# NazirNayal8/RbA

Hardware: AMD Instinct MI355X
Metric: images/sec @1024x2048 Swin-B-1dl (RbA inference hot path) (higher is better)
Workload: dtype f32 (f16x3 split-MFMA GEMMs, fp32 accumulate)

## Files before the change

include/rba_hip.h:

```cpp
#ifndef RBA_HIP_H
#define RBA_HIP_H

#include <stdint.h>

#ifdef __cplusplus
extern "C" {
#endif

int rba_hip_version(void);

int rba_set_concurrent_streams(int n);

int rba_reduce_f32(const float* mask, const float* cls_prob, float* rba, float* sem_seg, int32_t* argmax,
                   int Q, int K, int64_t HW, int score_mode, void* stream);

int rba_reduce_ws_f32(const float* mask, const float* cls_prob, float* rba, float* sem_seg, int32_t* argmax, int Q, int K,
                      int64_t HW, int score_mode, void* workspace, void* stream);

int rba_reduce_up4_f32(const float* mask_lowres, const float* cls_prob, float* rba, float* sem_seg,
                       int32_t* argmax, int Q, int K, int h, int w, int crop_h, int crop_w, int score_mode, void* stream);

int rba_reduce_bwd_workspace_f32(int Q, int K, int64_t HW, int64_t* bytes);
int rba_reduce_bwd_f32(const float* mask, const float* cls_prob, const float* grad_score,
                       float* grad_mask , float* grad_prob ,
// ... 127 lines not shown
                                        int rows_per_image, void* stream);

int rba_split_linear_nchw_out_gn_f16x3_f32(const float* x, const float* mr, const float* gamma, const float* beta, int G, int relu,
                                           const void* weight_packed, const float* bias, float* out, int64_t M, int N, int K,
                                           int rows_per_image, void* stream);

int rba_split_linear_nchw_out_gn_rows_f16x3_f32(const float* x, const float* mr, const float* gamma, const float* beta, int G, int relu,
                                                const void* weight_packed, int64_t weight_image_stride, const float* bias,
                                                int bias_image_stride, const int32_t* row_index, float* out, int B, int P, int R, int N,
                                                int K, void* stream);
int rba_compose_query_operand_f16x2(const float* embed, const float* weight, const float* bias, void* packed, float* bias_q, int B, int Q,
                                    int C, int K, void* stream);

int rba_conv3x3_nhwc_f32(const float* x, const void* weight_packed, const float* bias, float* out, int B, int H, int W, int C,
                         int N, void* stream);

int rba_conv3x3_nhwc_f16x3_f32(const float* x, const void* weight_packed, const float* bias, float* out, int B, int H, int W, int C,
                               int N, void* stream);

int rba_split_linear_f16x3_gn_moments_f32(const float* x, const void* weight_packed, const float* bias, float* out, int64_t M, int N, int K,
                                          int rows_per_image, int G, float* moments, void* stream);
int rba_conv3x3_nhwc_f16x3_split_in_gn_moments_f32(const void* x_frag, const void* weight_packed, const float* bias, float* out, int B, int H,
                                                   int W, int C, int N, int G, float* moments, void* stream);
int rba_group_norm_nhwc_merge_f32(const float* moments, float* mr, int B, int G, int splits, float eps, void* stream);

int rba_patch_im2col_u8(const uint8_t* image, float* out, int h, int w, int Hp, int Wp, const float* mean, const float* std, void* stream);
int rba_patch_im2col_f32(const float* image, float* out, int h, int w, int Hp, int Wp, const float* mean, const float* std, void* stream);

int rba_gaussian_blur_f32(const float* in, float* out, int H, int W, int kernel_size, float sigma, void* stream);

int rba_quad_mean_f32(const float* v, float* out, int64_t rows, int S, void* stream);
int rba_softmax_drop_last_f32(const float* logits, float* prob, int64_t rows, int K1, void* stream);

int rba_threshold_u8(const float* score, uint8_t* out, int64_t n, float threshold, void* stream);
int rba_morph3x3_u8(const uint8_t* in, uint8_t* out, int H, int W, int dilate, void* stream);
int rba_ccl4_roots_i32(const uint8_t* mask, int32_t* roots, int H, int W, void* stream);

int rba_bn_relu_conv1x1_f32(const float* x, const float* scale, const float* shift, const float* weight, const float* bias, float* out,
                            int B, int C, int O, int64_t P, void* stream);
int rba_resample_bilinear_ac_f32(const float* x, float* out, int C, int h, int w, int H, int W, void* stream);

typedef struct {
  const float* x_add;
  const void* packed;
  const float* bias;
  float* out;
// ... 15 lines not shown
```

rba_amd/_lib.py:

```python
import ctypes
import os

_HERE = os.path.dirname(os.path.abspath(__file__))
LIB_PATH = os.environ.get("RBA_HIP_LIB") or os.path.join(_HERE, "csrc", "librba_hip.so")
KNOBS_LIB_PATH = os.path.join(_HERE, "csrc", "librba_hip_knobs.so")

_i = ctypes.c_int
_i64 = ctypes.c_int64
_vp = ctypes.c_void_p

SIGNATURES = {
    "rba_hip_version": [],
    "rba_set_concurrent_streams": [_i],
    "rba_reduce_f32": [_vp, _vp, _vp, _vp, _vp, _i, _i, _i64, _i, _vp],
    "rba_reduce_ws_f32": [_vp, _vp, _vp, _vp, _vp, _i, _i, _i64, _i, _vp, _vp],
    "rba_reduce_up4_f32": [_vp, _vp, _vp, _vp, _vp, _i, _i, _i, _i, _i, _i, _i, _vp],
    "rba_reduce_bwd_workspace_f32": [_i, _i, _i64, _vp],
    "rba_reduce_bwd_f32": [_vp, _vp, _vp, _vp, _vp, _i, _i, _i64, _i, _vp, _i64, _vp],
    "rba_resample_bilinear_f32": [_vp, _vp, _vp, _i, _i, _i, _i, _i, _vp],
    "rba_ms_deform_attn_fwd_f32": [_vp, _vp, _vp, _vp, _vp, _vp, _i, _i, _i, _i, _i, _i, _i, _vp],
    "rba_ms_deform_attn_fwd_f64": [_vp, _vp, _vp, _vp, _vp, _vp, _i, _i, _i, _i, _i, _i, _i, _vp],
    "rba_ms_deform_attn_bwd_f32": [_vp, _vp, _vp, _vp, _vp, _vp, _vp, _vp, _vp, _i, _i, _i, _i, _i, _i, _i, _vp],
    "rba_ms_deform_attn_bwd_f64": [_vp, _vp, _vp, _vp, _vp, _vp, _vp, _vp, _vp, _i, _i, _i, _i, _i, _i, _i, _vp],
    "rba_msda_prepare_f32": [_vp, _vp, _vp, _vp, _vp, _i64, _i, _i, _i, _vp],
# ... 16 lines not shown
    "rba_swin_bias_fragments_elems": [_i, _i],
    "rba_swin_attn_block_supported": [_i, _i],
    "rba_swin_attn_block_weight_bytes": [_i],
    "rba_swin_attn_qkv_supported": [_i, _i],
    "rba_swin_attn_qkv_split_out_f32": [_vp, _vp, _vp, _vp, ctypes.c_float, _vp, _vp, _vp, _i, _i, _i, _i, _i, _i, _vp],
    "rba_swin_attn_block_pack_f32": [_vp, _vp, _vp, _i, _vp],
    "rba_swin_attn_block_f32": [_vp, _vp, _vp, _vp, ctypes.c_float, _vp, _vp, _vp, _vp, _vp, _vp, ctypes.c_float, _i, _i, _i, _i, _i, _i, _vp],
    "rba_swin_bias_fragments_f32": [_vp, _vp, _i, _i, _vp],
    "rba_skinny_linear_f32": [_vp, _vp, _vp, _vp, _i, _i, _i, _i, _vp],
    "rba_skinny_linear_add_f32": [_vp, _vp, _i, _vp, _vp, _vp, _i, _i, _i, _i, _i, _vp],
    "rba_split_weight_bf16x3": [_vp, _vp, _i, _i, _vp],
    "rba_split_linear_f32": [_vp, _vp, _vp, _vp, _i64, _i, _i, _i, _vp],
    "rba_split_weight_f16x2": [_vp, _vp, _i, _i, _vp],
    "rba_split_linear_f16x3_f32": [_vp, _vp, _vp, _vp, _i64, _i, _i, _i, _vp],
    "rba_split_linear_f16x3_res_f32": [_vp, _vp, _vp, _vp, _vp, _i64, _i, _i, _vp],
    "rba_split_linear_f16x3_frag_f32": [_vp, _vp, _vp, _vp, _vp, _i64, _i, _i, _i, _vp],
    "rba_swin_mlp_fused_f16x3_f32": [_vp, _vp, _vp, _vp, _vp, _vp, _vp, _i64, _i, _i, _vp],
    "rba_swin_mlp_fused_ln_f16x3_f32": [_vp, _vp, _vp, ctypes.c_float, _vp, _vp, _vp, _vp, _i64, _i, _i, _vp],
    "rba_split_linear_f16x3_gelu_split_out": [_vp, _i, _vp, _vp, _vp, _i64, _i, _i, _vp],
    "rba_split_linear_nchw_out_f32": [_vp, _vp, _vp, _vp, _i64, _i, _i, _i, _vp],
    "rba_split_linear_nchw_out_f16x3_f32": [_vp, _vp, _vp, _vp, _i64, _i, _i, _i, _vp],
    "rba_split_linear_f16x3_gn_moments_f32": [_vp, _vp, _vp, _vp, _i64, _i, _i, _i, _i, _vp, _vp],
    "rba_conv3x3_nhwc_f16x3_split_in_gn_moments_f32": [_vp, _vp, _vp, _vp, _i, _i, _i, _i, _i, _i, _vp, _vp],
    "rba_group_norm_nhwc_merge_f32": [_vp, _vp, _i, _i, _i, ctypes.c_float, _vp],
    "rba_split_linear_nchw_out_gn_f16x3_f32": [_vp, _vp, _vp, _vp, _i, _i, _vp, _vp, _vp, _i64, _i, _i, _i, _vp],
    "rba_split_linear_nchw_out_gn_rows_f16x3_f32": [_vp, _vp, _vp, _vp, _i, _i, _vp, _i64, _vp, _i, _vp, _vp, _i, _i, _i, _i, _i, _vp],
    "rba_compose_query_operand_f16x2": [_vp, _vp, _vp, _vp, _vp, _i, _i, _i, _i, _vp],
    "rba_conv3x3_nhwc_f32": [_vp, _vp, _vp, _vp, _i, _i, _i, _i, _i, _vp],
    "rba_conv3x3_nhwc_f16x3_f32": [_vp, _vp, _vp, _vp, _i, _i, _i, _i, _i, _vp],
    "rba_conv3x3_nhwc_f16x3_split_in_f32": [_vp, _vp, _vp, _vp, _i, _i, _i, _i, _i, _vp],
    "rba_resample_bilinear_nhwc_split_out_f32": [_vp, _vp, _vp, _i, _i, _i, _i, _i, _i64, _vp],
    "rba_patch_im2col_u8": [_vp, _vp, _i, _i, _i, _i, _vp, _vp, _vp],
    "rba_patch_im2col_f32": [_vp, _vp, _i, _i, _i, _i, _vp, _vp, _vp],
    "rba_group_norm_nhwc_workspace_bytes": [_i, _i, _i, _i],
    "rba_group_norm_nhwc_f32": [_vp, _vp, _vp, _vp, _vp, _i, _i, _i, _i, ctypes.c_float, _i, _vp],
    "rba_resample_bilinear_nhwc_f32": [_vp, _vp, _vp, _i, _i, _i, _i, _i, _vp],
    "rba_bn_relu_conv1x1_f32": [_vp, _vp, _vp, _vp, _vp, _vp, _i, _i, _i, _i64, _vp],
    "rba_resample_bilinear_ac_f32": [_vp, _vp, _i, _i, _i, _i, _i, _vp],
    "rba_gaussian_blur_f32": [_vp, _vp, _i, _i, _i, ctypes.c_float, _vp],
    "rba_quad_mean_f32": [_vp, _vp, _i64, _i, _vp],
    "rba_softmax_drop_last_f32": [_vp, _vp, _i64, _i, _vp],
    "rba_threshold_u8": [_vp, _vp, _i64, ctypes.c_float, _vp],
    "rba_morph3x3_u8": [_vp, _vp, _i, _i, _i, _vp],
    "rba_ccl4_roots_i32": [_vp, _vp, _i, _i, _vp],
    "rba_add_layer_norm_f32": [_vp, _vp, _vp, _vp, _vp, _vp, _vp, _i64, _i, ctypes.c_float, _vp],
    "rba_add_layer_norm_frag_f32": [_vp, _vp, _vp, _vp, _vp, _vp, _vp, _i64, _i, ctypes.c_float, _vp],
# ... 96 lines not shown
```

rba_amd/csrc/group_norm.hip:

```cpp
#include "common.h"
#include "../../include/rba_hip.h"

namespace {

constexpr int CHUNK = 16384;

__device__ __forceinline__ double wave_sum_d(double v) {
#pragma unroll
  for (int o = 32; o > 0; o >>= 1) v += __shfl_xor(v, o, RBA_WAVE);
  return v;
}

__global__ __launch_bounds__(256) void gn_stats_kernel(const float* __restrict__ x, float* __restrict__ ws, int64_t gsize,
                                                       int splits) {
  const int s = blockIdx.x, g = blockIdx.y;
  const int64_t lo = (int64_t)s * CHUNK, hi = lo + CHUNK < gsize ? lo + CHUNK : gsize;
  const float* p = x + (int64_t)g * gsize;
  float sum = 0.f, sq = 0.f;
  if ((gsize & 3) == 0 && (((uintptr_t)p) & 15) == 0) {
    for (int64_t i = lo + threadIdx.x * 4; i < hi; i += 1024) {
      const float4 v = *reinterpret_cast<const float4*>(p + i);
      sum += (v.x + v.y) + (v.z + v.w);
      sq = fmaf(v.x, v.x, sq); sq = fmaf(v.y, v.y, sq); sq = fmaf(v.z, v.z, sq); sq = fmaf(v.w, v.w, sq);
    }
// ... 77 lines not shown
    for (int p = lo + pl; p < hi; p += lanes) {
      const float4 v = xp[(int64_t)p * C4];
      sum += (v.x + v.y) + (v.z + v.w);
      sq = fmaf(v.x, v.x, sq); sq = fmaf(v.y, v.y, sq); sq = fmaf(v.z, v.z, sq); sq = fmaf(v.w, v.w, sq);
    }
  __shared__ float sh_s[256], sh_q[256];
  sh_s[threadIdx.x] = sum;
  sh_q[threadIdx.x] = sq;
  __syncthreads();
  const int G = C / cpg, q4 = cpg >> 2;
  if (threadIdx.x < G) {
    const int g = threadIdx.x;
    double ds = 0, dq = 0;
    for (int l = 0; l < lanes; ++l)
      for (int k = 0; k < q4; ++k) { ds += sh_s[l * C4 + g * q4 + k]; dq += sh_q[l * C4 + g * q4 + k]; }
    const double n = (double)(hi - lo) * cpg;
    const double mean = ds / n;
    const double m2 = dq - ds * mean;
    float* o = ws + (((int64_t)b * G + g) * splits + s) * 3;
    o[0] = (float)n; o[1] = (float)mean; o[2] = (float)(m2 > 0 ? m2 : 0);
  }
}

__global__ __launch_bounds__(64) void gn_merge_kernel(const float* __restrict__ ws, float* __restrict__ mr, int splits, float eps) {
  const float* w = ws + (int64_t)blockIdx.x * splits * 3;
  double n = 0, nm = 0;
  for (int i = threadIdx.x; i < splits; i += 64) { n += w[3 * i]; nm += (double)w[3 * i] * w[3 * i + 1]; }
  n = wave_sum_d(n); nm = wave_sum_d(nm);
  const double mean = nm / n;
  double m2 = 0;
  for (int i = threadIdx.x; i < splits; i += 64) {
    const double d = (double)w[3 * i + 1] - mean;
    m2 += (double)w[3 * i + 2] + (double)w[3 * i] * d * d;
  }
  m2 = wave_sum_d(m2);
  if (threadIdx.x == 0) { mr[2 * blockIdx.x] = (float)mean; mr[2 * blockIdx.x + 1] = (float)(1.0 / sqrt(m2 / n + (double)eps)); }
}

template <bool RELU>
__global__ __launch_bounds__(256) void gn_apply_nhwc_kernel(const float* __restrict__ x, const float* __restrict__ mr,
                                                            const float* __restrict__ gamma, const float* __restrict__ beta,
                                                            float* __restrict__ y, int P, int C, int cpg) {
  const int s = blockIdx.x, b = blockIdx.y;
  const int C4 = C >> 2, lanes = 256 / C4;
  const int j = threadIdx.x % C4, pl = threadIdx.x / C4;
  if (pl >= lanes) return;
  const int G = C / cpg, g = (j << 2) / cpg;
  const float mean = mr[2 * (b * G + g)], rstd = mr[2 * (b * G + g) + 1];
  const float4 ga = reinterpret_cast<const float4*>(gamma)[j], be = reinterpret_cast<const float4*>(beta)[j];
  const float a0 = ga.x * rstd, a1 = ga.y * rstd, a2 = ga.z * rstd, a3 = ga.w * rstd;
  const float b0 = fmaf(-mean, a0, be.x), b1 = fmaf(-mean, a1, be.y), b2 = fmaf(-mean, a2, be.z), b3 = fmaf(-mean, a3, be.w);
  const int lo = s * PIX_CHUNK, hi = lo + PIX_CHUNK < P ? lo + PIX_CHUNK : P;
  const float4* xp = reinterpret_cast<const float4*>(x + (int64_t)b * P * C) + j;
  float4* yp = reinterpret_cast<float4*>(y + (int64_t)b * P * C) + j;
#pragma unroll 8
  for (int p = lo + pl; p < hi; p += lanes) {
    float4 v = xp[(int64_t)p * C4];
    v.x = fmaf(v.x, a0, b0); v.y = fmaf(v.y, a1, b1); v.z = fmaf(v.z, a2, b2); v.w = fmaf(v.w, a3, b3);
    if (RELU) { v.x = rba_relu(v.x); v.y = rba_relu(v.y); v.z = rba_relu(v.z); v.w = rba_relu(v.w); }
// ... 29 lines not shown
    hipLaunchKernelGGL(gn_apply_kernel<false>, grid, dim3(256), 0, st, x, workspace, gamma, beta, y, gsize, (int)splits, HW, cpg, G, eps);
  return rba_launch_status();
}

extern "C" int64_t rba_group_norm_nhwc_workspace_bytes(int B, int P, int C, int G) {
  if (B <= 0 || C <= 0 || P <= 0 || G <= 0 || C % G) return 0;
  const int64_t splits = (P + PIX_CHUNK - 1) / PIX_CHUNK;
  return ((int64_t)B * G * splits * 3 + (int64_t)B * G * 2) * (int64_t)sizeof(float);
}

extern "C" int rba_group_norm_nhwc_f32(const float* x, const float* gamma, const float* beta, float* y, float* workspace, int B,
                                       int P, int C, int G, float eps, int relu, void* stream) {
  RBA_CHECK_ARG(B >= 0 && C >= 4 && P >= 0 && G >= 1 && C % G == 0 && (C / G) % 4 == 0 && C <= 1024 && 256 % (C / 4) == 0 && G <= 256);
  if (B == 0 || P == 0) return 0;
  RBA_CHECK_ARG(x && gamma && beta && y && workspace && B <= 65535);
  RBA_CHECK_ARG((((uintptr_t)x | (uintptr_t)y | (uintptr_t)gamma | (uintptr_t)beta) & 15) == 0);
  const int cpg = C / G;
  const int splits = (P + PIX_CHUNK - 1) / PIX_CHUNK;
  float* mr = workspace + (int64_t)B * G * splits * 3;
  rba_begin();
  hipStream_t st = (hipStream_t)stream;
  const dim3 grid(splits, B);
  hipLaunchKernelGGL(gn_stats_nhwc_kernel, grid, dim3(256), 0, st, x, workspace, P, C, cpg, splits);
  hipLaunchKernelGGL(gn_merge_kernel, dim3(B * G), dim3(64), 0, st, workspace, mr, splits, eps);
  if (relu)
    hipLaunchKernelGGL(gn_apply_nhwc_kernel<true>, grid, dim3(256), 0, st, x, mr, gamma, beta, y, P, C, cpg);
  else
    hipLaunchKernelGGL(gn_apply_nhwc_kernel<false>, grid, dim3(256), 0, st, x, mr, gamma, beta, y, P, C, cpg);
  return rba_launch_status();
}

extern "C" int rba_group_norm_nhwc_stats_f32(const float* x, float* mr, float* workspace, int B, int P, int C, int G, float eps, void* stream) {
  RBA_CHECK_ARG(B >= 0 && C >= 4 && P >= 0 && G >= 1 && C % G == 0 && (C / G) % 4 == 0 && C <= 1024 && 256 % (C / 4) == 0 && G <= 256);
  if (B == 0 || P == 0) return 0;
  RBA_CHECK_ARG(x && mr && workspace && B <= 65535 && (((uintptr_t)x) & 15) == 0);
  const int splits = (P + PIX_CHUNK - 1) / PIX_CHUNK;
  rba_begin();
  hipStream_t st = (hipStream_t)stream;
  hipLaunchKernelGGL(gn_stats_nhwc_kernel, dim3(splits, B), dim3(256), 0, st, x, workspace, P, C, C / G, splits);
  hipLaunchKernelGGL(gn_merge_kernel, dim3(B * G), dim3(64), 0, st, workspace, mr, splits, eps);
  return rba_launch_status();
}

extern "C" int rba_group_norm_nhwc_merge_f32(const float* moments, float* mr, int B, int G, int splits, float eps, void* stream) {
  RBA_CHECK_ARG(B >= 0 && G >= 1 && splits >= 1 && (int64_t)B * G <= 0x7fffffff);
  if (B == 0) return 0;
  RBA_CHECK_ARG(moments && mr);
  rba_begin();
  hipLaunchKernelGGL(gn_merge_kernel, dim3(B * G), dim3(64), 0, (hipStream_t)stream, moments, mr, splits, eps);
  return rba_launch_status();
}
```

rba_amd/csrc/split_linear_dma.hip:

```cpp
#include "split_linear_h3.h"
#include "split_linear_h3q.h"
#include "mlp_fused_h3.h"

RBA_KNOB(rba_k6_variant, 0);
RBA_KNOB_DEFINE(rba_k6_stagger, 0);
RBA_KNOB_DEFINE(rba_k6_occ, 2);
RBA_KNOB_DEFINE(rba_k6_rs_min_k, 512);
RBA_KNOB_DEFINE(rba_k6_ks, 0);
RBA_KNOB_DEFINE(rba_k6_rs, 0);
extern "C" __attribute__((visibility("hidden"))) int rba_concurrent_streams_hint = 1;

extern "C" int rba_set_concurrent_streams(int n) {
  const int prev = rba_concurrent_streams_hint;
  rba_concurrent_streams_hint = n >= 1 ? n : 1;
  return prev;
}

extern "C" int rba_split_linear_f32(const float* x, const void* weight_planes, const float* bias, float* out, int64_t M, int N,
                                    int K, int act, void* stream) {
  RBA_CHECK_ARG(N >= 1 && act >= 0 && act <= 2);
  RBA_GEMM_PROLOGUE(M, K, x && weight_planes && out, x, weight_planes, out);
  const u32x4_t* wp = reinterpret_cast<const u32x4_t*>(weight_planes);
  hipStream_t st = (hipStream_t)stream;
  return rba_gemm_status((tiles128(M, N) < 256 && N > 64 && (K >> 5) >= 2) ? launch_v5_act<1, 2, 2, 2, 4>(act, x, wp, bias, out, M, N, K, 2, st)
// ... 77 lines not shown
  return rba_launch_status();
}

extern "C" int rba_split_linear_f16x3_f32(const float* x, const void* weight_packed, const float* bias, float* out, int64_t M, int N,
                                          int K, int act, void* stream) {
  RBA_CHECK_ARG(N >= 1 && act >= 0 && act <= 2);
  RBA_GEMM_PROLOGUE(M, K, x && weight_packed && out, x, weight_packed, out);
  const H3Args a{x, reinterpret_cast<const u32x4_t*>(weight_packed), bias, out, M, N, K, (hipStream_t)stream};
  return rba_gemm_status(h3_with_act(act, [&](auto ACT) { return launch_h3_rows<ACT, 0>(a); }));
}

extern "C" int rba_conv3x3_nhwc_f16x3_f32(const float* x, const void* weight_packed, const float* bias, float* out, int B, int H, int W,
                                          int C, int N, void* stream) {
  RBA_CHECK_ARG(B >= 0 && H >= 1 && W >= 1 && N >= 1);
  const int64_t M = (int64_t)B * H * W;
  RBA_GEMM_PROLOGUE(M, C, x && weight_packed && out && M * C < (int64_t)1 << 30, x, weight_packed, out);
  H3Args a{x, reinterpret_cast<const u32x4_t*>(weight_packed), bias, out, M, N, 9 * C, (hipStream_t)stream};
  a.cs = ConvShape{H, W, C};
  return rba_gemm_status((tiles128(M, N) >= 256 || N <= 64) ? launch_h3l<0, 4, H3_CONV>(a) : launch_h3l<0, 2, H3_CONV>(a));
}

extern "C" int rba_split_linear_f16x3_gn_moments_f32(const float* x, const void* weight_packed, const float* bias, float* out, int64_t M, int N, int K,
                                                     int rows_per_image, int G, float* moments, void* stream) {
  RBA_CHECK_ARG(N >= 128 && (N % 128) == 0 && K <= 256 && G >= 1 && (N % G) == 0 && rows_per_image >= 128);
  const int cpg = N / G;
  RBA_CHECK_ARG((cpg == 4 || cpg == 8 || cpg == 16 || cpg == 32) && (rows_per_image % 128) == 0);
  RBA_GEMM_PROLOGUE(M, K, x && weight_packed && out && moments && (M % rows_per_image) == 0, x, weight_packed, out);
  H3Args a{x, reinterpret_cast<const u32x4_t*>(weight_packed), bias, out, M, N, K, (hipStream_t)stream};
  a.gm = GnMoments{moments, G, cpg, rows_per_image};
  return rba_gemm_status(launch_h3l<0, 4, H3_GNM>(a));
}

extern "C" int rba_conv3x3_nhwc_f16x3_split_in_gn_moments_f32(const void* x_frag, const void* weight_packed, const float* bias, float* out, int B, int H,
                                                              int W, int C, int N, int G, float* moments, void* stream) {
  RBA_CHECK_ARG(B >= 0 && H >= 1 && W >= 1 && C <= 2048 && N >= 128 && (N % 128) == 0 && G >= 1 && (N % G) == 0);
  const int cpg = N / G;
  const int64_t P = (int64_t)H * W, M = (int64_t)B * P;
  RBA_CHECK_ARG((cpg == 4 || cpg == 8 || cpg == 16 || cpg == 32) && (P % 128) == 0 && P < (int64_t)1 << 31);
  RBA_GEMM_PROLOGUE(M, C, x_frag && weight_packed && out && moments, x_frag, weight_packed, out, bias);
  H3Args a{x_frag, reinterpret_cast<const u32x4_t*>(weight_packed), bias, out, M, N, 9 * C, (hipStream_t)stream};
  a.cs = ConvShape{H, W, C};
  a.gm = GnMoments{moments, G, cpg, (int)P};
  return rba_gemm_status(launch_h3p_by_shape<0, H3_PRE | H3_CONVP | H3_GNM, H3_RS2>(a));
}

extern "C" int rba_split_linear_f16x3_res_f32(const float* x, const void* weight_packed, const float* bias, const float* residual, float* out,
                                              int64_t M, int N, int K, void* stream) {
  RBA_CHECK_ARG(N >= 1);
  RBA_GEMM_PROLOGUE(M, K, x && weight_packed && residual && out, x, weight_packed, out, residual);
  H3Args a{x, reinterpret_cast<const u32x4_t*>(weight_packed), bias, out, M, N, K, (hipStream_t)stream};
  a.res = residual;
  return rba_gemm_status(launch_h3_rows<0, H3_RES>(a));
}
// ... 84 lines not shown
```

rba_amd/csrc/split_linear_h3.h:

```cpp
#pragma once
#include <type_traits>

#include "split_linear_dma.h"

RBA_KNOB_EXTERN(rba_k6_stagger, 0);

namespace {

typedef _Float16 f16x8_t __attribute__((ext_vector_type(8)));

__device__ __forceinline__ void split_h3(const f32x4 u, const f32x4 v, f16x8_t& h, f16x8_t& l) {
  const float x[8] = {u.x, u.y, u.z, u.w, v.x, v.y, v.z, v.w};
  u32x4_t hp, lp;
#pragma unroll
  for (int i = 0; i < 4; ++i) {
    uint32_t a, r;
    rba_split_f16x2(x[2 * i], x[2 * i + 1], a, r);
    hp[i] = a;
    lp[i] = r;
  }
  h = __builtin_bit_cast(f16x8_t, hp);
  l = __builtin_bit_cast(f16x8_t, lp);
}

// ... 173 lines not shown
  H3_PRE = 1u << 6,
  H3_FOUT = 1u << 7,
  H3_CONVP = 1u << 8,
  H3_OCC1 = 1u << 9,
  H3_KS2 = 1u << 10,
  H3_RS2 = 1u << 11,
  H3_ROWIDX = 1u << 12,
  H3_PERIMG = 1u << 13,
  H3_PROBE_SHIFT = 16,
};
constexpr unsigned h3_probe(int p) { return (unsigned)p << H3_PROBE_SHIFT; }
constexpr int h3_probe_of(unsigned form) { return (int)(form >> H3_PROBE_SHIFT); }
constexpr unsigned H3_FORMS = H3_TIMING | H3_RES, H3L_FORMS = H3_FORMS | H3_GNM | H3_CONV | H3_NCHW | H3_GNF | H3_ROWIDX | H3_PERIMG,
                   H3P_FORMS = H3_FORMS | H3_GNM | H3_PRE | H3_FOUT | H3_CONVP | H3_OCC1 | H3_KS2 | H3_RS2;
constexpr bool h3_form_within(unsigned form, unsigned allowed) { return (form & ~allowed & ((1u << H3_PROBE_SHIFT) - 1)) == 0; }
constexpr int h3_tile_rows(unsigned form) { return (form & H3_RS2) ? 256 : 128; }
constexpr int h3_threads(unsigned form) { return (form & (H3_KS2 | H3_RS2)) ? 512 : 256; }
constexpr int h3_occupancy(unsigned form) { return (form & (H3_KS2 | H3_RS2 | H3_OCC1)) ? 1 : 2; }

template <int ACT, int CT, unsigned FORM = 0>
__global__ __launch_bounds__(256, 2) void split_linear_h3_kernel(const float* __restrict__ A, const u32x4_t* __restrict__ Wp,
                                                                const float* __restrict__ bias, float* C, int M, int N,
                                                                int K, int MT, int NT, unsigned long long* dbg = nullptr,
                                                                const float* R = nullptr) {
  static_assert(h3_form_within(FORM, H3_FORMS), "split_linear_h3_kernel: H3_TIMING, H3_RES, h3_probe()");
  constexpr int PROBE = h3_probe_of(FORM);
  constexpr bool TIMING = FORM & H3_TIMING, RES = FORM & H3_RES;
  unsigned long long tm[4];
  if (TIMING) tm[0] = wall_clock64();
  constexpr int BM = 128, BN = 32 * CT;
  constexpr int SUBW = 4 * BN;
  constexpr int BLK = 2 * SUBW;
  constexpr int UPL = BLK / 256;
  static_assert(BLK % 256 == 0 && 128 % BN == 0, "tile width");
  __shared__ __attribute__((aligned(16))) u32x4_t lds[2 * BLK];

  const int tid = threadIdx.x, lane = tid & 63;
  const int wave = __builtin_amdgcn_readfirstlane(tid >> 6);
  int bid = blockIdx.x;
  const int nb = MT * NT;
  if ((nb & 7) == 0) bid = (bid & 7) * (nb >> 3) + (bid >> 3);
  const int mt = bid / NT, nt = bid - mt * NT;
  const int m0 = mt * BM, n0 = nt * BN;
  const int NB = K >> 5, S16 = K >> 4;
  const int l31 = lane & 31, lh = lane >> 5;

  constexpr int QSTEP = (CT == 4) ? 256 : 512;
  const char* wbase = reinterpret_cast<const char*>(Wp + (int64_t)(n0 >> 7) * S16 * 512 + (n0 & 127) * 2);
  uint32_t woff;
  {
// ... 64 lines not shown
#pragma unroll
      for (int j = 0; j < CT; ++j) accl[j] = __builtin_amdgcn_mfma_f32_32x32x16_f16(ah[g], bl[j], accl[j], 0, 0, 0);
#pragma unroll
      for (int j = 0; j < CT; ++j) accl[j] = __builtin_amdgcn_mfma_f32_32x32x16_f16(al[g], bh[j], accl[j], 0, 0, 0);
    }
    if (!(PROBE & 64)) asm volatile("s_waitcnt lgkmcnt(0)\n\ts_barrier" ::: "memory");
  };
  int b = 0;
  if (NB & 1) {
    block(0, lds, lds + BLK, xr[0]);
    b = 1;
    for (; b < NB; b += 2) {
      block(b, lds + BLK, lds, xr[1]);
      block(b + 1, lds, lds + BLK, xr[0]);
    }
  } else {
    for (; b < NB; b += 2) {
      block(b, lds, lds + BLK, xr[0]);
      block(b + 1, lds + BLK, lds, xr[1]);
    }
  }

  if (TIMING) tm[2] = wall_clock64();
  h3_epilogue<ACT, CT, PROBE, RES>(accm, accl, bias, C, R, M, N, m0, n0, BM, BN, wave, l31, lh);
  if (TIMING && tid == 0) {
    tm[3] = wall_clock64();
    unsigned xcc;
    asm volatile("s_getreg_b32 %0, hwreg(HW_REG_XCC_ID)" : "=s"(xcc));
    unsigned hw;
    asm volatile("s_getreg_b32 %0, hwreg(HW_REG_HW_ID)" : "=s"(hw));
#pragma unroll
    for (int i = 0; i < 4; ++i) dbg[6 * blockIdx.x + i] = tm[i];
    dbg[6 * blockIdx.x + 4] = xcc;
    dbg[6 * blockIdx.x + 5] = hw;
  }
}

struct ConvShape {
  int H, W, Cin;
};
struct GnFold {
  const float* mr;
  const float* gamma;
  const float* beta;
  int G, cpg, relu;
};
struct H3Rows {
// ... 543 lines not shown
  hipStream_t stream;
  const float* res = nullptr;
  unsigned long long* dbg = nullptr;
  ConvShape cs = ConvShape{0, 0, 0};
  int rows_per_image = 0;
  GnFold gn = GnFold{nullptr, nullptr, nullptr, 1, 1, 0};
  GnMoments gm = GnMoments{nullptr, 1, 1, 128};
  int stagger = 0;
  H3Rows rw = H3Rows{nullptr, 0, 0, 0};
};

inline bool h3_grid(const H3Args& a, int rows, int cols, int& MT, int& NT) {
  const int64_t mt = (a.M + rows - 1) / rows;
  MT = (int)mt;
  NT = (a.N + cols - 1) / cols;
  return mt * NT < (int64_t)1 << 31;
}

template <int ACT, int CT, unsigned FORM = 0>
int launch_h3(const H3Args& a) {
  int MT, NT;
  if (!h3_grid(a, 128, 32 * CT, MT, NT)) return (int)hipErrorInvalidValue;
  hipLaunchKernelGGL((split_linear_h3_kernel<ACT, CT, FORM>), dim3((unsigned)MT * NT), dim3(256), 0, a.stream, reinterpret_cast<const float*>(a.x), a.wp, a.bias,
                     reinterpret_cast<float*>(a.out), (int)a.M, a.N, a.K, MT, NT, a.dbg, a.res);
  return 0;
}

template <int ACT, int CT, unsigned FORM = 0>
int launch_h3l(const H3Args& a) {
  int MT, NT;
  if (!h3_grid(a, 128, 32 * CT, MT, NT)) return (int)hipErrorInvalidValue;
  hipLaunchKernelGGL((split_linear_h3l_kernel<ACT, CT, FORM>), dim3((unsigned)MT * NT), dim3(256), 0, a.stream, reinterpret_cast<const float*>(a.x), a.wp, a.bias,
                     reinterpret_cast<float*>(a.out), (int)a.M, a.N, a.K, MT, NT, a.dbg, a.cs, a.res, a.rows_per_image, a.gn, a.gm, a.rw);
  return 0;
}

template <int ACT, unsigned FORM = 0>
int launch_h3p(const H3Args& a) {
  int MT, NT;
  if (!h3_grid(a, h3_tile_rows(FORM), 128, MT, NT)) return (int)hipErrorInvalidValue;
  hipLaunchKernelGGL((split_linear_h3p_kernel<ACT, FORM>), dim3((unsigned)MT * NT), dim3(h3_threads(FORM)), 0, a.stream, reinterpret_cast<const float*>(a.x), a.wp,
                     a.bias, reinterpret_cast<float*>(a.out), (int)a.M, a.N, a.K, MT, NT, a.dbg, a.res, a.cs, h3_threads(FORM) == 256 ? a.stagger : 0, a.gm);
  return 0;
}

template <class F>
int h3_with_act(int act, F&& f) {
// ... 64 lines not shown
```

rba_amd/modeling/pixel_decoder/msdeformattn.py:

```python
import os

import torch
import torch.nn as nn
import torch.nn.functional as F

from ... import ops
from ...arch import FEATURE_NAMES, feature_channels, num_fpn_levels
from ...lru import ShapeCache, derived, source_key
from ...registry import SEM_SEG_HEADS_REGISTRY
from ..transformer_decoder.position_encoding import PositionEmbeddingSine
from .ops.ms_deform_attn import MSDeformAttn

FOLD_MASK_FEATURE_NORM = os.environ.get("RBA_MF_GN_FOLD", "1") != "0"


class DeferredMaskFeatures:

    def __init__(self, prev, mr, norm, conv, planes, hw, num_groups=32, relu=True):
        self.prev, self.mr, self.norm, self.conv, self.planes, self.hw = prev, mr, norm, conv, planes, hw
        self.num_groups, self.relu = num_groups, relu
        self.batch = mr.shape[0]
        self._tensor = None

    @property
# ... 192 lines not shown
        srcs, pos, tks = [], [], []
        for idx, f in enumerate(self.transformer_in_features[::-1]):
            x = features[f]
            B, _, h, w = x.shape
            conv, gn = self.input_proj[idx][0], self.input_proj[idx][1]
            y = ops.group_norm_nhwc(self._conv1x1(self._tokens(x), conv), 32, gn.weight, gn.bias, gn.eps)
            tks.append(y.view(B, h * w, -1))
            srcs.append(y.view(B, h, w, -1).permute(0, 3, 1, 2))
            pos.append(self.pe_layer(x))
        y, shapes = self.transformer(srcs, pos, tokens=tks)
        B, d = y.shape[0], y.shape[2]
        toks = [z.contiguous() for z in torch.split(y, [h * w for h, w in shapes], dim=1)]
        outs = [z.view(B, h, w, d).permute(0, 3, 1, 2) for z, (h, w) in zip(toks, shapes)]
        prev, (ph, pw) = toks[-1], shapes[-1]
        prev_norm = None
        fold = self.fold_group_norm
        for idx, f in enumerate(self.in_features[:self.num_fpn_levels][::-1]):
            j = self.num_fpn_levels - idx
            x = features[f]
            h, w = int(x.shape[-2]), int(x.shape[-1])
            ad, ly = getattr(self, f"adapter_{j}"), getattr(self, f"layer_{j}")
            tok = self._tokens(x)
            lat_mr = None
            if fold and tok.is_contiguous() and ops.linear_emits_gn_moments(B * h * w, d, tok.shape[-1], h * w, 32):
                lat, lat_mr = ops.linear_gn_stats(tok, _cached_linear_view(ad), 32, ad.norm.eps, h * w, use_bias=False)
            else:
                lat = self._conv1x1(tok, ad, use_bias=False)
            split = ops.conv3x3_takes_split(B * h * w, d) and d % 32 == 0
            yy = ops.SplitActivations.empty((B, h, w, d), prev.device) if split else None
            if fold:
                if lat_mr is None:
                    lat_mr = ops.group_norm_nhwc_stats(lat, 32, ad.norm.eps)
                ups = []
                for b in range(B):
                    xn = None if prev_norm is None else (prev_norm[0][b], prev_norm[1].weight, prev_norm[1].bias, True)
                    r = ops.resample_bilinear_nhwc_gn(prev[b].view(ph, pw, d), (h, w), lat[b].view(h, w, d), 32, x_norm=xn,
                                                      add_norm=(lat_mr[b], ad.norm.weight, ad.norm.bias), split_into=yy, image=b)
                    if not split:
                        ups.append(r)
                if not split:
                    yy = ups[0][None] if B == 1 else torch.stack(ups)
            else:
                if prev_norm is not None:
                    prev = ops.group_norm_nhwc(prev, 32, prev_norm[1].weight, prev_norm[1].bias, prev_norm[1].eps, relu=True)
                cur = ops.group_norm_nhwc(lat, 32, ad.norm.weight, ad.norm.bias, ad.norm.eps)
                if split:
                    for b in range(B):
                        ops.resample_bilinear_nhwc(prev[b].view(ph, pw, d), (h, w), add=cur[b].view(h, w, d), split_into=yy, image=b)
                else:
                    ups = [ops.resample_bilinear_nhwc(prev[b].view(ph, pw, d), (h, w), add=cur[b].view(h, w, d))
                           for b in range(B)]
                    yy = ups[0][None] if B == 1 else torch.stack(ups)
            planes = _conv3x3_planes(ly)
            last = idx == self.num_fpn_levels - 1
            if fold and split and ops.conv3x3_emits_gn_moments(B, h, w, d, 32):
                prev, mr = ops.conv3x3_nhwc_gn_stats(yy, planes, 32, ly.norm.eps, None, out_features=d)
                prev_norm = (mr, ly.norm)
                prev = prev.view(B, h * w, d)
            else:
                prev = ops.conv3x3_nhwc(yy, planes, None, out_features=d).view(B, h * w, d)
                prev_norm = (ops.group_norm_nhwc_stats(prev, 32, ly.norm.eps) if fold and not last else None, ly.norm)
            ph, pw = h, w
        mfw = self.mask_features.weight
        planes = derived(self.mask_features, ("mf_planes", ops.SPLIT_MODE), (mfw, self.mask_features.bias),
                         lambda: ops.split_weight(mfw.detach().view(mfw.shape[0], -1).contiguous()))
        if prev_norm is not None and fold and FOLD_MASK_FEATURE_NORM and ops.split_linear_nchw_out_takes_gn(planes, ph * pw, d, 32):
            mr = prev_norm[0] if prev_norm[0] is not None else ops.group_norm_nhwc_stats(prev, 32, prev_norm[1].eps)
            mf = DeferredMaskFeatures(prev.view(B * ph * pw, d), mr, prev_norm[1], self.mask_features, planes, (ph, pw), num_groups=32, relu=True)
            if not defer_mask_features:
                mf = mf.materialize()
            return mf, outs[0], outs[:self.maskformer_num_feature_levels]
        if prev_norm is not None:
            prev = ops.group_norm_nhwc(prev, 32, prev_norm[1].weight, prev_norm[1].bias, prev_norm[1].eps, relu=True)
        mf = ops.split_linear_nchw_out(prev.view(B * ph * pw, d), planes, self.mask_features.bias, ph * pw,
                                       out_features=mfw.shape[0]).view(B, mfw.shape[0], ph, pw)
        return mf, outs[0], outs[:self.maskformer_num_feature_levels]

    def forward_features(self, features, defer_mask_features=False):
# ... 20 lines not shown
```

rba_amd/ops.py:

```python
import contextlib
import ctypes
import threading
import functools
import math
import os

import torch

from . import _lib
from ._lib import RbaHipError
from .lru import derived


def _stream():
    return torch.cuda.current_stream().cuda_stream


def _launch(name, *args, stream=None):
    code = getattr(_lib.load(), name)(*args, torch.cuda.current_stream().cuda_stream if stream is None else stream)
    if code:
        _lib.check(code, name)


def _query(name, *args):
# ... 895 lines not shown
        raise RbaHipError("SplitActivations need f16x3 planes")
    out = torch.empty(lead + (N,), dtype=torch.float32, device=x.device)
    if pre:
        _launch("rba_split_linear_f16x3_frag_f32", xp, _p(planes), _p(bias), 0, _p(out), M, N, K, act)
    else:
        _launch("rba_split_linear_f16x3_f32" if f16 else "rba_split_linear_f32", xp, _p(planes), _p(bias), _p(out), M, N, K, act)
    return out


@_hip_op
def split_linear_nchw_out(x, planes, bias, rows_per_image, out_features=None):
    _chk(x, "x", dim=2)
    M, K = x.shape
    N, f16 = _packed(planes, K, out_features)
    if rows_per_image < 1 or M % rows_per_image:
        raise RbaHipError("split_linear_nchw_out needs x [B*P, K] with M % rows_per_image == 0")
    _vec(bias, "bias", N, optional=True)
    out = torch.empty((M // rows_per_image, N, rows_per_image), dtype=torch.float32, device=x.device)
    _launch("rba_split_linear_nchw_out_f16x3_f32" if f16 else "rba_split_linear_nchw_out_f32", _p(x), _p(planes), _p(bias), _p(out), M, N, K, rows_per_image)
    return out


GN_MOMENTS = os.environ.get("RBA_GN_MOMENTS", "1") != "0"


def _gn_moments_ok(rows_per_image, N, num_groups):
    return (GN_MOMENTS and _split_mode() == "f16x3" and rows_per_image % 128 == 0 and N % 128 == 0 and N % num_groups == 0
            and (N // num_groups) in (4, 8, 16, 32))


def linear_emits_gn_moments(M, N, K, rows_per_image, num_groups):
    return _gn_moments_ok(rows_per_image, N, num_groups) and K <= 256 and K % 32 == 0 and _tiles128(M, N) >= 160 and M % rows_per_image == 0


def conv3x3_emits_gn_moments(B, H, W, N, num_groups):
    return _gn_moments_ok(H * W, N, num_groups) and conv3x3_takes_split(B * H * W, N)


def _merge_gn_moments(moments, B, G, splits, eps):
    mr = torch.empty((B, G, 2), dtype=torch.float32, device=moments.device)
    _launch("rba_group_norm_nhwc_merge_f32", _p(moments), _p(mr), B, G, splits, float(eps))
    return mr


@_hip_op
def linear_gn_stats(x, lin, num_groups, eps, rows_per_image, use_bias=True):
    _chk(x, "x")
    w = lin.weight
    N, K = w.shape
    M = x.numel() // K
    if not linear_emits_gn_moments(M, N, K, rows_per_image, num_groups) or x.shape[-1] != K:
        raise RbaHipError("linear_gn_stats: check linear_emits_gn_moments(M, N, K, rows_per_image, G) first")
    bias = lin.bias if use_bias else None
    planes = _cached_planes(lin, w)
    B, splits = M // rows_per_image, rows_per_image // 128
    out = torch.empty(tuple(x.shape[:-1]) + (N,), dtype=torch.float32, device=x.device)
    mom = torch.empty((B, num_groups, splits, 3), dtype=torch.float32, device=x.device)
    _launch("rba_split_linear_f16x3_gn_moments_f32", _p(x), _p(planes), _p(bias), _p(out), M, N, K, rows_per_image, int(num_groups), _p(mom))
    return out, _merge_gn_moments(mom, B, int(num_groups), splits, eps)


@_hip_op
def conv3x3_nhwc_gn_stats(x, planes, num_groups, eps, bias=None, out_features=None):
    if not isinstance(x, SplitActivations):
        raise RbaHipError("conv3x3_nhwc_gn_stats needs SplitActivations of logical shape [B,H,W,C]")
    xp, _ = _split_x(x, "conv3x3_nhwc_gn_stats", dim=4)
    B, H, W, C = x.shape
    N, _ = _packed(planes, 9 * C, out_features, bf16x6=False)
    if C % 32 or not conv3x3_emits_gn_moments(B, H, W, N, num_groups):
        raise RbaHipError("conv3x3_nhwc_gn_stats: check conv3x3_emits_gn_moments(B, H, W, N, G) first")
    _vec(bias, "bias", N, optional=True)
    splits = H * W // 128
    out = torch.empty((B, H, W, N), dtype=torch.float32, device=x.device)
    mom = torch.empty((B, num_groups, splits, 3), dtype=torch.float32, device=x.device)
    _launch("rba_conv3x3_nhwc_f16x3_split_in_gn_moments_f32", xp, _p(planes), _p(bias), _p(out), B, H, W, C, N, int(num_groups), _p(mom))
    return out, _merge_gn_moments(mom, B, int(num_groups), splits, eps)


def split_linear_nchw_out_takes_gn(planes, rows_per_image, K, num_groups):
    return planes.dtype == torch.float16 and rows_per_image % 128 == 0 and K % num_groups == 0 and (K // num_groups) % 4 == 0 and K % 32 == 0


@_hip_op
def split_linear_nchw_out_gn(x, mr, weight, bias_gn, num_groups, relu, planes, bias, rows_per_image, out_features=None):
    _chk(x, "x", dim=2)
    _chk(mr, "mr", dim=3)
    M, K = x.shape
    N, _ = _packed(planes, K, out_features, bf16x6=False)
    if rows_per_image < 1 or M % rows_per_image or not split_linear_nchw_out_takes_gn(planes, rows_per_image, K, num_groups):
        raise RbaHipError("split_linear_nchw_out_gn needs x [B*P, K], P % 128 == 0 and (K / G) % 4 == 0")
    B = M // rows_per_image
    if tuple(mr.shape) != (B, num_groups, 2):
        raise RbaHipError("mr must be [B, G, 2]")
    _vec(weight, "weight", K)
    _vec(bias_gn, "bias_gn", K)
    _vec(bias, "bias", N, optional=True)
    out = torch.empty((B, N, rows_per_image), dtype=torch.float32, device=x.device)
    _launch("rba_split_linear_nchw_out_gn_f16x3_f32", _p(x), _p(mr), _p(weight), _p(bias_gn), int(num_groups), int(bool(relu)), _p(planes), _p(bias), _p(out),
# ... 382 lines not shown
```

Measured before the change: 149.8.

## Extend GroupNorm moment fusion to narrow GEMMs, fp32-row conv3x3, and unrolled merge

Lets the f16x3 linear and conv3x3 GEMM epilogues emit GroupNorm partial moments in more cases: N multiples of 64, K above 256 through the non-DMA kernel, and conv3x3 on plain fp32 rows rather than only split activations. The pixel decoder routes more adapter and layer convs through these fused paths, so fewer separate GN statistics passes over the output are needed. The merge kernel now batches its loads with a template unroll and reuses them when one pass covers all splits. The trade-off is that smaller tile shapes carry epilogue overhead and may lose occupancy on narrow layers.

New measurement: 150.0 (median of 5 runs). No clear change (+0.1%).

```diff
diff --git a/include/rba_hip.h b/include/rba_hip.h
--- a/include/rba_hip.h
+++ b/include/rba_hip.h
@@ -173,6 +173,8 @@
                                           int rows_per_image, int G, float* moments, void* stream);
 int rba_conv3x3_nhwc_f16x3_split_in_gn_moments_f32(const void* x_frag, const void* weight_packed, const float* bias, float* out, int B, int H,
                                                    int W, int C, int N, int G, float* moments, void* stream);
+int rba_conv3x3_nhwc_f16x3_gn_moments_f32(const float* x, const void* weight_packed, const float* bias, float* out, int B, int H, int W, int C, int N, int G,
+                                          float* moments, void* stream);
 int rba_group_norm_nhwc_merge_f32(const float* moments, float* mr, int B, int G, int splits, float eps, void* stream);
 
 int rba_patch_im2col_u8(const uint8_t* image, float* out, int h, int w, int Hp, int Wp, const float* mean, const float* std, void* stream);
diff --git a/rba_amd/_lib.py b/rba_amd/_lib.py
--- a/rba_amd/_lib.py
+++ b/rba_amd/_lib.py
@@ -62,6 +62,7 @@
     "rba_split_linear_nchw_out_f16x3_f32": [_vp, _vp, _vp, _vp, _i64, _i, _i, _i, _vp],
     "rba_split_linear_f16x3_gn_moments_f32": [_vp, _vp, _vp, _vp, _i64, _i, _i, _i, _i, _vp, _vp],
     "rba_conv3x3_nhwc_f16x3_split_in_gn_moments_f32": [_vp, _vp, _vp, _vp, _i, _i, _i, _i, _i, _i, _vp, _vp],
+    "rba_conv3x3_nhwc_f16x3_gn_moments_f32": [_vp, _vp, _vp, _vp, _i, _i, _i, _i, _i, _i, _vp, _vp],
     "rba_group_norm_nhwc_merge_f32": [_vp, _vp, _i, _i, _i, ctypes.c_float, _vp],
     "rba_split_linear_nchw_out_gn_f16x3_f32": [_vp, _vp, _vp, _vp, _i, _i, _vp, _vp, _vp, _i64, _i, _i, _i, _vp],
     "rba_split_linear_nchw_out_gn_rows_f16x3_f32": [_vp, _vp, _vp, _vp, _i, _i, _vp, _i64, _vp, _i, _vp, _vp, _i, _i, _i, _i, _i, _vp],
diff --git a/rba_amd/csrc/group_norm.hip b/rba_amd/csrc/group_norm.hip
--- a/rba_amd/csrc/group_norm.hip
+++ b/rba_amd/csrc/group_norm.hip
@@ -123,19 +123,65 @@
   }
 }
 
+template <int U>
+struct GnMergeBatch {
+  float n[U], m[U], q[U];
+};
+template <int U>
+__device__ __forceinline__ void gn_merge_load(GnMergeBatch<U>& t, const float* __restrict__ w, int splits, int i0) {
+#pragma unroll
+  for (int u = 0; u < U; ++u) {
+    int i = i0 + 64 * u;
+    i = i < splits ? i : splits - 1;
+    t.n[u] = w[3 * i];
+    t.m[u] = w[3 * i + 1];
+    t.q[u] = w[3 * i + 2];
+  }
+}
+template <int U>
+__device__ __forceinline__ void gn_merge_sum_n(const GnMergeBatch<U>& t, int splits, int i0, double& n, double& nm) {
+#pragma unroll
+  for (int u = 0; u < U; ++u)
+    if (i0 + 64 * u < splits) {
+      n += t.n[u];
+      nm += (double)t.n[u] * t.m[u];
+    }
+}
+template <int U>
+__device__ __forceinline__ void gn_merge_sum_m2(const GnMergeBatch<U>& t, int splits, int i0, double mean, double& m2) {
+#pragma unroll
+  for (int u = 0; u < U; ++u)
+    if (i0 + 64 * u < splits) {
+      const double d = (double)t.m[u] - mean;
+      m2 += (double)t.q[u] + (double)t.n[u] * d * d;
+    }
+}
+template <int U>
 __global__ __launch_bounds__(64) void gn_merge_kernel(const float* __restrict__ ws, float* __restrict__ mr, int splits, float eps) {
   const float* w = ws + (int64_t)blockIdx.x * splits * 3;
+  const int lane = threadIdx.x;
+  const bool once = splits <= 64 * U;
+  GnMergeBatch<U> t;
   double n = 0, nm = 0;
-  for (int i = threadIdx.x; i < splits; i += 64) { n += w[3 * i]; nm += (double)w[3 * i] * w[3 * i + 1]; }
+  for (int i0 = lane; i0 < splits; i0 += 64 * U) {
+    gn_merge_load(t, w, splits, i0);
+    gn_merge_sum_n(t, splits, i0, n, nm);
+  }
   n = wave_sum_d(n); nm = wave_sum_d(nm);
   const double mean = nm / n;
   double m2 = 0;
-  for (int i = threadIdx.x; i < splits; i += 64) {
-    const double d = (double)w[3 * i + 1] - mean;
-    m2 += (double)w[3 * i + 2] + (double)w[3 * i] * d * d;
+  for (int i0 = lane; i0 < splits; i0 += 64 * U) {
+    if (!once) gn_merge_load(t, w, splits, i0);
+    gn_merge_sum_m2(t, splits, i0, mean, m2);
   }
   m2 = wave_sum_d(m2);
-  if (threadIdx.x == 0) { mr[2 * blockIdx.x] = (float)mean; mr[2 * blockIdx.x + 1] = (float)(1.0 / sqrt(m2 / n + (double)eps)); }
+  if (lane == 0) { mr[2 * blockIdx.x] = (float)mean; mr[2 * blockIdx.x + 1] = (float)(1.0 / sqrt(m2 / n + (double)eps)); }
+}
+
+static void launch_gn_merge(const float* ws, float* mr, int groups, int splits, float eps, hipStream_t st) {
+  if (splits <= 64) hipLaunchKernelGGL(gn_merge_kernel<1>, dim3(groups), dim3(64), 0, st, ws, mr, splits, eps);
+  else if (splits <= 256) hipLaunchKernelGGL(gn_merge_kernel<4>, dim3(groups), dim3(64), 0, st, ws, mr, splits, eps);
+  else hipLaunchKernelGGL(gn_merge_kernel<16>, dim3(groups), dim3(64), 0, st, ws, mr, splits, eps);
 }
 
 template <bool RELU>
@@ -211,7 +257,7 @@
   hipStream_t st = (hipStream_t)stream;
   const dim3 grid(splits, B);
   hipLaunchKernelGGL(gn_stats_nhwc_kernel, grid, dim3(256), 0, st, x, workspace, P, C, cpg, splits);
-  hipLaunchKernelGGL(gn_merge_kernel, dim3(B * G), dim3(64), 0, st, workspace, mr, splits, eps);
+  launch_gn_merge(workspace, mr, B * G, splits, eps, st);
   if (relu)
     hipLaunchKernelGGL(gn_apply_nhwc_kernel<true>, grid, dim3(256), 0, st, x, mr, gamma, beta, y, P, C, cpg);
   else
@@ -227,7 +273,7 @@
   rba_begin();
   hipStream_t st = (hipStream_t)stream;
   hipLaunchKernelGGL(gn_stats_nhwc_kernel, dim3(splits, B), dim3(256), 0, st, x, workspace, P, C, C / G, splits);
-  hipLaunchKernelGGL(gn_merge_kernel, dim3(B * G), dim3(64), 0, st, workspace, mr, splits, eps);
+  launch_gn_merge(workspace, mr, B * G, splits, eps, st);
   return rba_launch_status();
 }
 
@@ -236,6 +282,6 @@
   if (B == 0) return 0;
   RBA_CHECK_ARG(moments && mr);
   rba_begin();
-  hipLaunchKernelGGL(gn_merge_kernel, dim3(B * G), dim3(64), 0, (hipStream_t)stream, moments, mr, splits, eps);
-  return rba_launch_status();
-}
+  launch_gn_merge(moments, mr, B * G, splits, eps, (hipStream_t)stream);
+  return rba_launch_status();
+}
diff --git a/rba_amd/csrc/split_linear_dma.hip b/rba_amd/csrc/split_linear_dma.hip
--- a/rba_amd/csrc/split_linear_dma.hip
+++ b/rba_amd/csrc/split_linear_dma.hip
@@ -123,13 +123,29 @@
 
 extern "C" int rba_split_linear_f16x3_gn_moments_f32(const float* x, const void* weight_packed, const float* bias, float* out, int64_t M, int N, int K,
                                                      int rows_per_image, int G, float* moments, void* stream) {
-  RBA_CHECK_ARG(N >= 128 && (N % 128) == 0 && K <= 256 && G >= 1 && (N % G) == 0 && rows_per_image >= 128);
+  RBA_CHECK_ARG(N >= 64 && (N % 64) == 0 && G >= 1 && (N % G) == 0 && rows_per_image >= 128);
   const int cpg = N / G;
   RBA_CHECK_ARG((cpg == 4 || cpg == 8 || cpg == 16 || cpg == 32) && (rows_per_image % 128) == 0);
+  const bool wide = h3_wide(M, N) && (N % 128) == 0;
+  RBA_CHECK_ARG(K <= 256 || !wide);
   RBA_GEMM_PROLOGUE(M, K, x && weight_packed && out && moments && (M % rows_per_image) == 0, x, weight_packed, out);
   H3Args a{x, reinterpret_cast<const u32x4_t*>(weight_packed), bias, out, M, N, K, (hipStream_t)stream};
   a.gm = GnMoments{moments, G, cpg, rows_per_image};
-  return rba_gemm_status(launch_h3l<0, 4, H3_GNM>(a));
+  if (K > 256) return rba_gemm_status(launch_h3<0, 2, H3_GNM>(a));
+  return rba_gemm_status(wide ? launch_h3l<0, 4, H3_GNM>(a) : launch_h3l<0, 2, H3_GNM>(a));
+}
+
+extern "C" int rba_conv3x3_nhwc_f16x3_gn_moments_f32(const float* x, const void* weight_packed, const float* bias, float* out, int B, int H, int W, int C, int N,
+                                                     int G, float* moments, void* stream) {
+  RBA_CHECK_ARG(B >= 0 && H >= 1 && W >= 1 && N >= 64 && (N % 64) == 0 && G >= 1 && (N % G) == 0);
+  const int cpg = N / G;
+  const int64_t P = (int64_t)H * W, M = (int64_t)B * P;
+  RBA_CHECK_ARG((cpg == 4 || cpg == 8 || cpg == 16 || cpg == 32) && (P % 128) == 0 && P < (int64_t)1 << 31 && tiles128(M, N) < 256);
+  RBA_GEMM_PROLOGUE(M, C, x && weight_packed && out && moments && M * C < (int64_t)1 << 30, x, weight_packed, out);
+  H3Args a{x, reinterpret_cast<const u32x4_t*>(weight_packed), bias, out, M, N, 9 * C, (hipStream_t)stream};
+  a.cs = ConvShape{H, W, C};
+  a.gm = GnMoments{moments, G, cpg, (int)P};
+  return rba_gemm_status(launch_h3l<0, 2, H3_CONV | H3_GNM>(a));
 }
 
 extern "C" int rba_conv3x3_nhwc_f16x3_split_in_gn_moments_f32(const void* x_frag, const void* weight_packed, const float* bias, float* out, int B, int H,
diff --git a/rba_amd/csrc/split_linear_h3.h b/rba_amd/csrc/split_linear_h3.h
--- a/rba_amd/csrc/split_linear_h3.h
+++ b/rba_amd/csrc/split_linear_h3.h
@@ -219,10 +219,10 @@
 __global__ __launch_bounds__(256, 2) void split_linear_h3_kernel(const float* __restrict__ A, const u32x4_t* __restrict__ Wp,
                                                                 const float* __restrict__ bias, float* C, int M, int N,
                                                                 int K, int MT, int NT, unsigned long long* dbg = nullptr,
-                                                                const float* R = nullptr) {
-  static_assert(h3_form_within(FORM, H3_FORMS), "split_linear_h3_kernel: H3_TIMING, H3_RES, h3_probe()");
+                                                                const float* R = nullptr, GnMoments gm = GnMoments{nullptr, 1, 1, 128}) {
+  static_assert(h3_form_within(FORM, H3_FORMS | H3_GNM), "split_linear_h3_kernel: H3_TIMING, H3_RES, H3_GNM, h3_probe()");
   constexpr int PROBE = h3_probe_of(FORM);
-  constexpr bool TIMING = FORM & H3_TIMING, RES = FORM & H3_RES;
+  constexpr bool TIMING = FORM & H3_TIMING, RES = FORM & H3_RES, GNM = FORM & H3_GNM;
   unsigned long long tm[4];
   if (TIMING) tm[0] = wall_clock64();
   constexpr int BM = 128, BN = 32 * CT;
@@ -333,7 +333,7 @@
   }
 
   if (TIMING) tm[2] = wall_clock64();
-  h3_epilogue<ACT, CT, PROBE, RES>(accm, accl, bias, C, R, M, N, m0, n0, BM, BN, wave, l31, lh);
+  h3_epilogue<ACT, CT, PROBE, RES, GNM>(accm, accl, bias, C, R, M, N, m0, n0, BM, BN, wave, l31, lh, gm, reinterpret_cast<float*>(lds));
   if (TIMING && tid == 0) {
     tm[3] = wall_clock64();
     unsigned xcc;
@@ -923,7 +923,7 @@
   int MT, NT;
   if (!h3_grid(a, 128, 32 * CT, MT, NT)) return (int)hipErrorInvalidValue;
   hipLaunchKernelGGL((split_linear_h3_kernel<ACT, CT, FORM>), dim3((unsigned)MT * NT), dim3(256), 0, a.stream, reinterpret_cast<const float*>(a.x), a.wp, a.bias,
-                     reinterpret_cast<float*>(a.out), (int)a.M, a.N, a.K, MT, NT, a.dbg, a.res);
+                     reinterpret_cast<float*>(a.out), (int)a.M, a.N, a.K, MT, NT, a.dbg, a.res, a.gm);
   return 0;
 }
 
diff --git a/rba_amd/modeling/pixel_decoder/msdeformattn.py b/rba_amd/modeling/pixel_decoder/msdeformattn.py
--- a/rba_amd/modeling/pixel_decoder/msdeformattn.py
+++ b/rba_amd/modeling/pixel_decoder/msdeformattn.py
@@ -238,7 +238,8 @@
             ad, ly = getattr(self, f"adapter_{j}"), getattr(self, f"layer_{j}")
             tok = self._tokens(x)
             lat_mr = None
-            if fold and tok.is_contiguous() and ops.linear_emits_gn_moments(B * h * w, d, tok.shape[-1], h * w, 32):
+            if (fold and tok.is_contiguous() and ops.linear_emits_gn_moments(B * h * w, d, tok.shape[-1], h * w, 32)
+                    and (ops.split_linear_pays(B * h * w, d, tok.shape[-1]) or not ops.token_linear_pays(B * h * w, d, tok.shape[-1]))):
                 lat, lat_mr = ops.linear_gn_stats(tok, _cached_linear_view(ad), 32, ad.norm.eps, h * w, use_bias=False)
             else:
                 lat = self._conv1x1(tok, ad, use_bias=False)
@@ -269,7 +270,8 @@
                     yy = ups[0][None] if B == 1 else torch.stack(ups)
             planes = _conv3x3_planes(ly)
             last = idx == self.num_fpn_levels - 1
-            if fold and split and ops.conv3x3_emits_gn_moments(B, h, w, d, 32):
+            if fold and (ops.conv3x3_emits_gn_moments(B, h, w, d, 32) if split else
+                         planes.dtype == torch.float16 and ops.conv3x3_rows_emit_gn_moments(B, h, w, d, 32)):
                 prev, mr = ops.conv3x3_nhwc_gn_stats(yy, planes, 32, ly.norm.eps, None, out_features=d)
                 prev_norm = (mr, ly.norm)
                 prev = prev.view(B, h * w, d)
diff --git a/rba_amd/ops.py b/rba_amd/ops.py
--- a/rba_amd/ops.py
+++ b/rba_amd/ops.py
@@ -941,19 +941,28 @@
 
 
 GN_MOMENTS = os.environ.get("RBA_GN_MOMENTS", "1") != "0"
-
-
-def _gn_moments_ok(rows_per_image, N, num_groups):
-    return (GN_MOMENTS and _split_mode() == "f16x3" and rows_per_image % 128 == 0 and N % 128 == 0 and N % num_groups == 0
-            and (N // num_groups) in (4, 8, 16, 32))
+GN_MOMENTS_64 = os.environ.get("RBA_GN_MOMENTS_64", "1") != "0"
+
+
+def _gn_moments_ok(rows_per_image, N, num_groups, tile=128):
+    return (GN_MOMENTS and (tile == 128 or GN_MOMENTS_64) and _split_mode() == "f16x3" and rows_per_image % 128 == 0 and N % tile == 0
+            and N % num_groups == 0 and (N // num_groups) in (4, 8, 16, 32))
 
 
 def linear_emits_gn_moments(M, N, K, rows_per_image, num_groups):
-    return _gn_moments_ok(rows_per_image, N, num_groups) and K <= 256 and K % 32 == 0 and _tiles128(M, N) >= 160 and M % rows_per_image == 0
+    if K % 32 or M % rows_per_image:
+        return False
+    if _tiles128(M, N) >= 160 and N % 128 == 0:
+        return _gn_moments_ok(rows_per_image, N, num_groups) and K <= 256
+    return _gn_moments_ok(rows_per_image, N, num_groups, tile=64)
 
 
 def conv3x3_emits_gn_moments(B, H, W, N, num_groups):
     return _gn_moments_ok(H * W, N, num_groups) and conv3x3_takes_split(B * H * W, N)
+
+
+def conv3x3_rows_emit_gn_moments(B, H, W, N, num_groups):
+    return _gn_moments_ok(H * W, N, num_groups, tile=64) and _tiles128(B * H * W, N) < 256
 
 
 def _merge_gn_moments(moments, B, G, splits, eps):
@@ -981,18 +990,17 @@
 
 @_hip_op
 def conv3x3_nhwc_gn_stats(x, planes, num_groups, eps, bias=None, out_features=None):
-    if not isinstance(x, SplitActivations):
-        raise RbaHipError("conv3x3_nhwc_gn_stats needs SplitActivations of logical shape [B,H,W,C]")
-    xp, _ = _split_x(x, "conv3x3_nhwc_gn_stats", dim=4)
+    xp, pre = _split_x(x, "conv3x3_nhwc_gn_stats", dim=4)
     B, H, W, C = x.shape
     N, _ = _packed(planes, 9 * C, out_features, bf16x6=False)
-    if C % 32 or not conv3x3_emits_gn_moments(B, H, W, N, num_groups):
-        raise RbaHipError("conv3x3_nhwc_gn_stats: check conv3x3_emits_gn_moments(B, H, W, N, G) first")
+    if C % 32 or not (conv3x3_emits_gn_moments if pre else conv3x3_rows_emit_gn_moments)(B, H, W, N, num_groups):
+        raise RbaHipError("conv3x3_nhwc_gn_stats: check conv3x3_emits_gn_moments(B, H, W, N, G) (SplitActivations) / conv3x3_rows_emit_gn_moments (fp32 rows) first")
     _vec(bias, "bias", N, optional=True)
     splits = H * W // 128
     out = torch.empty((B, H, W, N), dtype=torch.float32, device=x.device)
     mom = torch.empty((B, num_groups, splits, 3), dtype=torch.float32, device=x.device)
-    _launch("rba_conv3x3_nhwc_f16x3_split_in_gn_moments_f32", xp, _p(planes), _p(bias), _p(out), B, H, W, C, N, int(num_groups), _p(mom))
+    _launch("rba_conv3x3_nhwc_f16x3_split_in_gn_moments_f32" if pre else "rba_conv3x3_nhwc_f16x3_gn_moments_f32", xp, _p(planes), _p(bias), _p(out), B, H, W, C, N,
+            int(num_groups), _p(mom))
     return out, _merge_gn_moments(mom, B, int(num_groups), splits, eps)
 
 
```
